# chhylp123/hifiasm

Measured on AMD Instinct MI355X. Metric: read-pair overlaps/sec (sum ol->length / (ha_pt_gen + all-reads h_ec_lchain pass)), higher is better.
Workload: dtype u64 hashing / int32 + f64 chain scores

## Files before the change

hifiasm_amd/csrc/hao_batch.hpp:

```cpp
#pragma once
#include <sys/mman.h>
#include "hao_tables.hpp"
#include "hao_query.cuh"
#include "hao_query3.cuh"
#include "hao_query5.cuh"
#include "hao_grid.cuh"
#include "hao_chain.cuh"

struct hao_ctx::Batch {
	uint64_t n_generic = 0, n_generic_hits = 0, seed_path = 0, seed_left[3] = {0, 0, 0}; DevBuf<unsigned long long> stats, dbgbuf;
	uint64_t lo = 0, n = 0, mz0 = 0, n_mz = 0, n_anchor = 0, n_groups = 0, n_chains = 0, n_cl = 0, n_fc_raw = 0, n_ol = 0, n_fc = 0, n_fcw = 0;
	bool valid = false, host_valid = false;
	DevBuf<uint64_t> s_start, s_pk, a_off, seg, g_cnt, g_off, g_start, ch_base, cl_base, fc_base, fcs, fc_raw, ol_fc_off, cc_off, cc, fc_final, fcf_off;
	DevBuf<uint64_t> nch64;
	DevBuf<uint64_t> g_tmp, cls_cc, cls_co; DevBuf<hao_gent> glist; DevBuf<uint8_t> g_cls; DevBuf<uint32_t> slow, ovf_list; hipStream_t side[HAO_NCLS]; hipEvent_t ev_qc[HAO_NCLS], ev_dp[HAO_NCLS]; bool side_ready = false; hipEvent_t ev_pk0 = nullptr, ev_pk1 = nullptr; DevBuf<unsigned char> pk_tmp;
	DevBuf<uint32_t> q_pos, q_cnt, s_n, g_read, wgt, nch, nout, perm, n_final, fclen;
	DevBuf<hao_hit_t> hits, ohits, cl;
	DevBuf<int32_t> f, ii, p, key_sc, tm; DevBuf<int64_t> t; DevBuf<uint64_t> key_xs; DevBuf<uint32_t> key_al, key_tmp;
	DevBuf<hao_chain_rec> rec; DevBuf<hao_ovlp_t> ol; DevBuf<hao_cdesc> cd; bool cl_valid = false;
	DevBuf<uint16_t> hq, ohq; DevBuf<uint8_t> hcode;
	DevBuf<uint32_t> pk_cnt, pk_ecnt, pk_erank; uint64_t n_codes = 0;
	struct OutSet {
		DevBuf<hao_ovlp_t> ol_out; DevBuf<hao_ovlp_wire_t> ol_wire; DevBuf<uint64_t> fin_off, fc_out, fc_out_off, ch_off, cl_off, qm_off, fcw_off; DevBuf<uint32_t> fcw;
		DevBuf<hao_chain_hdr_t> hdr; DevBuf<uint64_t> bits; DevBuf<uint32_t> rank, rank4; DevBuf<uint8_t> codes; DevBuf<hao_exc_t> exc; DevBuf<hao_qmz_t> qmz; DevBuf<uint16_t> qmz_pos, qmz_cnt; bool qmz16 = false;
		DevBuf<uint8_t> exact;
		DevBuf<uint64_t> ed_off; DevBuf<uint8_t> ed_err; DevBuf<uint16_t> ed_pe;
		DevBuf<hao_ed_ovlp_sum> ed_sum;
		DevBuf<uint64_t> wl_woff, wl_cigoff; DevBuf<hao_rs_win> wl_wins; DevBuf<uint16_t> wl_cig;
		DevBuf<hao_rs_ovlp> rs_ovlp; DevBuf<uint64_t> rs_off; DevBuf<hao_rs_win> rs_wins;
		DevBuf<uint64_t> tr_off; DevBuf<uint16_t> tr_ps, tr_ncig, tr_cig;
	} out[2];
	int cur = 0;
	OutSet &O() { return out[cur]; }
	unsigned char *arena[2] = { nullptr, nullptr }; size_t arena_cap[2] = { 0, 0 }; bool arena_reg[2] = { false, false };
	void arena_free(int x) { if (!arena[x]) return; if (arena_reg[x]) { (void)hipHostUnregister(arena[x]); (void)munmap(arena[x], arena_cap[x]); } else (void)hipHostFree(arena[x]); arena[x] = nullptr; arena_cap[x] = 0; arena_reg[x] = false; } hipStream_t copy_stream = nullptr; hipEvent_t ev_ready[2], ev_done[2], ev_cstart[2]; bool arena_bad[2] = { false, false }; int arena_retry[2] = { 0, 0 }, arena_node = -1;       bool dl_ready = false, dl_pending[2] = { false, false };
	uint32_t wgt_hi = 0xffffffffu, wgt_lo = 0xffffffffu, wgt_max = 0xffffffffu;
	double t_evsync = 0, t_enq = 0, t_alloc = 0, t_s1 = 0, t_s2 = 0, t_s3 = 0, t_run = 0, t_pre = 0; uint64_t t_n = 0, t_nrun = 0;
	uint64_t ed_unres = 0;
	DevBuf<uint64_t> ed_nwin, ed_wbase, ed_wcnt, ed_woff; DevBuf<hao_ed_pair> ed_pairs; uint64_t ed_n = 0;
	hao_ed_delivery_t ed_dl[2] = {};
	uint64_t wl_cnt[5] = { 0, 0, 0, 0, 0 }; hao_wlist_delivery_t wl_dl[2] = {}; bool wl_on[2] = { false, false };
	uint64_t rs_nw = 0, rs_nres = 0, rs_wc = 0; hao_rescue_delivery_t rs_dl[2] = {}; bool rs_on[2] = { false, false };
	uint64_t tr_n = 0, tr_ncig = 0; hao_trace_delivery_t tr_dl[2] = {}; bool tr_on[2] = { false, false };
	hao_delivery_t dl[2]; uint64_t dl_seq = 0, n_exc = 0; uint32_t dl_parts = 0; bool exact_valid = false; std::vector<uint8_t> h_exact;
	std::vector<uint64_t> h_seg, h_fin_off, h_cl_off, h_fc_out_off; std::vector<hao_hit_t> h_hits, h_cl; std::vector<hao_ovlp_t> h_ol; std::vector<uint64_t> h_fc;
	std::vector<uint64_t> fetch_fc_off, h_cco;
	~Batch() {
		if (ev_pk0) { (void)hipEventDestroy(ev_pk0); (void)hipEventDestroy(ev_pk1); }
		if (side_ready) { for (int x = 0; x < HAO_NCLS; ++x) { (void)hipStreamDestroy(side[x]); (void)hipEventDestroy(ev_qc[x]); (void)hipEventDestroy(ev_dp[x]); } }
		if (dl_ready) { (void)hipStreamSynchronize(copy_stream); (void)hipStreamDestroy(copy_stream); for (int x = 0; x < 2; ++x) { (void)hipEventDestroy(ev_ready[x]); (void)hipEventDestroy(ev_done[x]); (void)hipEventDestroy(ev_cstart[x]); arena_free(x); } }
	}
};

__global__ void hao_cc_count_kernel(const uint32_t *len, uint64_t rid0, uint64_t n, uint64_t ocv_w, uint64_t *out)
{
	const uint64_t r = (uint64_t)blockIdx.x * blockDim.x + threadIdx.x;
	if (r > n) return;
// ... 492 lines not shown
		HIP_TRY(hipMemcpy(c->h_ix_mz_off.data(), c->d_ix_mz_off.p, (c->n_reads + 1) * 8, hipMemcpyDeviceToHost));
	}
	const uint64_t glo = c->rid_base + lo;
	B.mz0 = c->h_ix_mz_off[lo]; B.n_mz = c->h_ix_mz_off[hi] - B.mz0;
	const uint64_t nm = B.n_mz;
	if (B.wgt_hi != ps.high_occ || B.wgt_lo != ps.low_occ || !B.wgt.p) {
		std::vector<uint32_t> wt; hao_seed_weight_table(ps.high_occ, ps.low_occ, wt);
		HIP_TRY(B.wgt.reserve(4096)); HIP_TRY(hipMemcpy(B.wgt.p, wt.data(), 4096 * 4, hipMemcpyHostToDevice));
		B.wgt_hi = ps.high_occ; B.wgt_lo = ps.low_occ; B.wgt_max = *std::max_element(wt.begin(), wt.end());
	}
	HIP_TRY(B.q_pos.reserve(nm + 1)); HIP_TRY(B.q_cnt.reserve(nm + 1));
	HIP_TRY(B.s_start.reserve(nm + 1)); HIP_TRY(B.s_pk.reserve(nm + 1)); HIP_TRY(B.s_n.reserve(nm + 1)); HIP_TRY(B.a_off.reserve(nm + 2)); HIP_TRY(B.seg.reserve(n + 2));
	HIP_TRY(c->d_err.reserve(2)); HIP_TRY(hipMemsetAsync(c->d_err.p, 0, 4, c->stream));
	if (!c->lk_valid) { hao_set_err(c, "index without per-minimizer lookup results"); return HAO_EINVAL; }
	hipLaunchKernelGGL(seed_unpack_kernel, dim3((unsigned)((nm + 256) / 256)), dim3(256), 0, c->stream, c->d_ix_lk.p, c->d_ix_mz_info.p, B.mz0, nm, B.wgt.p, B.s_start.p, B.s_n.p, B.q_pos.p, B.q_cnt.p, B.s_pk.p);
	HAO_CHECK_LAUNCH();
	if (int rc = hao_scan_u32(c, B.s_n.p, B.a_off.p, nm + 1)) return rc;
	hipLaunchKernelGGL(seed_segments_kernel, dim3((unsigned)((n + 256) / 256)), dim3(256), 0, c->stream, c->d_ix_mz_off.p, lo, n, B.mz0, B.a_off.p, B.seg.p);
	HAO_CHECK_LAUNCH();
	hipLaunchKernelGGL(hao_peek_kernel, dim3(1), dim3(64), 0, c->stream, (const unsigned long long*)(B.a_off.p + nm), 1, c->peek_d);
	HAO_CHECK_LAUNCH();
	const double ts0_ = hao_now();
	HIP_TRY(hipStreamSynchronize(c->stream));
	B.t_s1 += hao_now() - ts0_; B.t_pre += ts0_ - t_run0;
	B.n_anchor = c->peek_h[0];
	c->timer.mark("q_lookup");
	const uint64_t A = B.n_anchor;
	if (A >= (1ULL << 32)) { hao_set_err(c, "batch produces >= 2^32 anchors: use a smaller read range"); return HAO_EUNSUPP; }
	HIP_TRY(B.hits.reserve(A + 1));
	uint64_t max_q = 1;
	for (uint64_t r = lo; r < hi; ++r) max_q = std::max<uint64_t>(max_q, c->h_ix_mz_off[r + 1] - c->h_ix_mz_off[r]);
	const uint64_t sum_q = c->h_ix_mz_off[hi] - c->h_ix_mz_off[lo];
	int tb = 1; while ((1ULL << tb) < c->n_total) ++tb;
	HIP_TRY(B.g_cnt.reserve(n + 2)); HIP_TRY(B.g_off.reserve(n + 2)); HIP_TRY(B.g_tmp.reserve(A + 1));
	HIP_TRY(B.stats.reserve(3 * HAO_NCLS + 7)); HIP_TRY(hipMemsetAsync(B.stats.p, 0, (3 * HAO_NCLS + 7) * 8, c->stream));
	unsigned long long *d_slow_cnt = B.stats.p, *d_cls_cnt = B.stats.p + HAO_NCLS + 4;
	{
		hao_seed_args sa_; B.seed_path = 0;
		sa_.mz_off = c->d_ix_mz_off.p; sa_.mz_info = c->d_ix_mz_info.p; sa_.rid_lo = lo; sa_.mz0 = B.mz0; sa_.s_start = B.s_start.p; sa_.s_n = B.s_n.p; sa_.a_off = B.a_off.p; sa_.seg = B.seg.p;
		sa_.sinfo = c->d_ix_sinfo.p; sa_.len = c->d_len_all.p; sa_.q_pos = B.q_pos.p; sa_.q_cnt = B.q_cnt.p; sa_.hits = B.hits.p; sa_.g_tmp = B.g_tmp.p; sa_.g_cnt = B.g_cnt.p; sa_.n_sel = n; sa_.tb = tb;
		sa_.qcap = (uint32_t)std::min<uint64_t>((max_q + 63) & ~63ULL, HAO_QTAB_CAP);
		sa_.dbg = nullptr; sa_.hq = nullptr;
		if (parts & HAO_DELIVER_CL) {
			HIP_TRY(B.hcode.reserve(A + 64));
			if (c->sw.seq_chain || c->sw.dp_seqtail || c->sw.dp_nospec) { const uint64_t n16 = (A + 31) / 16; hipLaunchKernelGGL(hao_fill16_kernel, dim3((unsigned)std::min<uint64_t>((n16 + 255) / 256, 1u << 14)), dim3(256), 0, c->stream, (hao_fill_v4*)B.hcode.p, n16, 0x08080808u); HAO_CHECK_LAUNCH(); }
			HIP_TRY(B.hq.reserve(A + 64)); sa_.hq = B.hq.p;
		}
		if (c->sw.seedphase) { HIP_TRY(B.dbgbuf.reserve(64)); HIP_TRY(hipMemsetAsync(B.dbgbuf.p, 0, 512, c->stream)); sa_.dbg = B.dbgbuf.p; }
		HIP_TRY(B.ovf_list.reserve(3 * (n + 1)));
		unsigned long long *d_ovf = B.stats.p + 3 * HAO_NCLS + 3, *d_ovf2 = B.stats.p + 3 * HAO_NCLS + 4, *d_ovf0 = B.stats.p + 3 * HAO_NCLS + 5;
		uint32_t *ovf1 = B.ovf_list.p, *ovf2 = B.ovf_list.p + (n + 1), *ovf0 = B.ovf_list.p + 2 * (n + 1);
		const size_t lds_tile = std::max<size_t>((size_t)512 * (sizeof(hao_stage_t) + 4), 12 * 512);
		const size_t lds_q = 12 * (size_t)sa_.qcap + 16;
		size_t lds1 = (size_t)22 * 512 + lds_tile + lds_q, lds2 = (size_t)22 * 1024 + std::max<size_t>(lds_tile, 12 * 1024) + lds_q,
			   lds3 = (size_t)22 * 2048 + std::max<size_t>(lds_tile, 12 * 2048) + lds_q;
		auto launch = [&](auto k1, auto k2, auto k3) -> int {
			{
				HIP_TRY(hipFuncSetAttribute((const void*)k1, hipFuncAttributeMaxDynamicSharedMemorySize, (int)lds1));
				HIP_TRY(hipFuncSetAttribute((const void*)k2, hipFuncAttributeMaxDynamicSharedMemorySize, (int)lds2));
				HIP_TRY(hipFuncSetAttribute((const void*)k3, hipFuncAttributeMaxDynamicSharedMemorySize, (int)lds3));
			}
			hipLaunchKernelGGL(k1, dim3((unsigned)n), dim3(256), lds1, c->stream, sa_, (const uint32_t*)nullptr, (const unsigned long long*)nullptr, ovf1, d_ovf);
			HAO_CHECK_LAUNCH();
			hipLaunchKernelGGL(k2, dim3((unsigned)n), dim3(256), lds2, c->stream, sa_, (const uint32_t*)ovf1, (const unsigned long long*)d_ovf, ovf2, d_ovf2);
			HAO_CHECK_LAUNCH();
			hipLaunchKernelGGL(k3, dim3((unsigned)n), dim3(256), lds3, c->stream, sa_, (const uint32_t*)ovf2, (const unsigned long long*)d_ovf2, (uint32_t*)nullptr, (unsigned long long*)nullptr);
			HAO_CHECK_LAUNCH();
// ... 103 lines not shown
			const hao_gent *lst0 = B.glist.p + L.base[0]; uint32_t *slow0 = B.slow.p + L.base[0];
			const unsigned nb_lane = (unsigned)std::min<uint64_t>((cls_cnt[0] + 63) / 64, 256 * 64);
			if (ca.dbg_seq == 1) hipLaunchKernelGGL(chain_tiny_kernel, dim3(nb_lane), dim3(64), 0, c->stream, ca, lst0, (uint64_t)cls_cnt[0], (const uint32_t*)nullptr, (const unsigned long long*)nullptr);
			else {
				hipLaunchKernelGGL(chain_pack8_kernel, dim3((unsigned)((cls_cnt[0] + 31) / 32)), dim3(256), 0, c->stream, ca, lst0, (uint64_t)cls_cnt[0], slow0);
				HAO_CHECK_LAUNCH();
				hipLaunchKernelGGL(chain_tiny_kernel, dim3(nb_lane), dim3(64), 0, c->stream, ca, lst0, (uint64_t)cls_cnt[0], (const uint32_t*)slow0, (const unsigned long long*)d_slow_cnt);
			}
			HAO_CHECK_LAUNCH();
		}
		if (ca.dbg_qc) { unsigned long long d_[5]; HIP_TRY(hipMemcpy(d_, B.dbgbuf.p, 40, hipMemcpyDeviceToHost)); if (d_[3]) fprintf(stderr, "[qc] fast groups %llu (avg %.0f hits)  avg us: entry + tile 0 %.2f  scan loop %.2f  cigar + record %.2f\n", d_[3], (double)d_[4] / d_[3], d_[0] / 100.0 / d_[3], d_[1] / 100.0 / d_[3], d_[2] / 100.0 / d_[3]); }
		c->timer.mark("q_chain");
		if (!serial) for (int x = 1; x < HAO_NCLS; ++x) if (cls_cnt[x]) HIP_TRY(hipStreamWaitEvent(c->stream, B.ev_dp[x], 0));
	}
	HIP_TRY(hipMemsetAsync(B.nch.p + G, 0, 4, c->stream)); HIP_TRY(hipMemsetAsync(B.nout.p + G, 0, 4, c->stream));
	c->timer.mark("q_chain_dp");
	HIP_TRY(B.ch_base.reserve(G + 2)); HIP_TRY(B.cl_base.reserve(G + 2)); HIP_TRY(B.fc_base.reserve(G * HAO_MCOPY_MAX + 2)); HIP_TRY(B.nch64.reserve(G * HAO_MCOPY_MAX + 2));
	if (int rc = hao_scan_u32(c, B.nch.p, B.ch_base.p, G + 1)) return rc;
	if (int rc = hao_scan_u32(c, B.nout.p, B.cl_base.p, G + 1)) return rc;
	hipLaunchKernelGGL(hao_fclen_kernel, dim3((unsigned)((G * HAO_MCOPY_MAX + 256) / 256)), dim3(256), 0, c->stream, B.rec.p, B.nch.p, G, B.nch64.p);
	HAO_CHECK_LAUNCH();
	if (int rc = hao_excl_scan_u64(c, B.nch64.p, B.fc_base.p, G * HAO_MCOPY_MAX + 1)) return rc;
	const uint64_t NCmax = G * HAO_MCOPY_MAX, FCmax = A + 6 * G;
	HIP_TRY(B.ol.reserve(NCmax + 1)); HIP_TRY(B.ol_fc_off.reserve(NCmax + 1)); HIP_TRY(B.cd.reserve(NCmax + 1)); HIP_TRY(B.fc_raw.reserve(FCmax + 1)); HIP_TRY(B.perm.reserve(NCmax + 1));
	if (G) {
		hao_asm_args aa;
		aa.g_start = B.g_start.p; aa.g_read = B.g_read.p; aa.g_cls = B.g_cls.p; aa.g_off = B.g_off.p; aa.n_groups = G; aa.rid_lo = glo; aa.ohits = B.ohits.p; aa.hits = B.hits.p; aa.fcs = B.fcs.p; aa.rec = B.rec.p; aa.nch = B.nch.p;
		aa.ch_base = B.ch_base.p; aa.cl_base = B.cl_base.p; aa.fc_base = B.fc_base.p; aa.ol = B.ol.p; aa.ol_fc_off = B.ol_fc_off.p; aa.cd = B.cd.p; aa.fc = B.fc_raw.p;
		hipLaunchKernelGGL(chain_assemble_kernel, dim3((unsigned)((G + 255) / 256)), dim3(256), 0, c->stream, aa); HAO_CHECK_LAUNCH();
	}
	unsigned long long *d_exc_cnt = B.stats.p + 3 * HAO_NCLS + 2;
	hao_pack_args pa; memset(&pa, 0, sizeof(pa));
	const uint64_t NW = (A + 63) / 64;
	unsigned long long *d_n_codes = B.stats.p + 3 * HAO_NCLS + 1;
	auto pack = [&](hipStream_t ps) -> int {
		if (!G) return HAO_OK;
		hao_ctx::Batch::OutSet &O = B.O();
		hipLaunchKernelGGL(hao_pack_hdr_kernel, dim3((unsigned)((NCmax + 255) / 256)), dim3(256), 0, ps, pa, B.ch_base.p + G); HAO_CHECK_LAUNCH();
		hipLaunchKernelGGL(hao_pack_bits_kernel, dim3((unsigned)((NW * 8 + 256 * HAO_PACK_U - 1) / (256 * HAO_PACK_U))), dim3(256), 0, ps, pa, A, NW, O.bits.p, B.pk_cnt.p, B.pk_ecnt.p); HAO_CHECK_LAUNCH();
		size_t tb = 0;
		HIP_TRY(rocprim::exclusive_scan(nullptr, tb, B.pk_cnt.p, O.rank.p, 0u, NW + 1, rocprim::plus<uint32_t>(), ps)); HIP_TRY(B.pk_tmp.reserve(tb + 256));
		HIP_TRY(rocprim::exclusive_scan(B.pk_tmp.p, tb, B.pk_cnt.p, O.rank.p, 0u, NW + 1, rocprim::plus<uint32_t>(), ps));
		HIP_TRY(rocprim::exclusive_scan(B.pk_tmp.p, tb, B.pk_ecnt.p, B.pk_erank.p, 0u, NW + 1, rocprim::plus<uint32_t>(), ps));
		hipLaunchKernelGGL(hao_pack_codes_kernel, dim3((unsigned)((NW * 8 + 255) / 256)), dim3(256), 0, ps, pa, B.hcode.p, A, O.bits.p, O.rank.p, NW, O.codes.p, d_n_codes, B.pk_erank.p); HAO_CHECK_LAUNCH();
		{ const uint64_t n4 = NW / 4 + 1; hipLaunchKernelGGL(hao_rank4_kernel, dim3((unsigned)((n4 + 255) / 256)), dim3(256), 0, ps, O.rank.p, n4, O.rank4.p); HAO_CHECK_LAUNCH(); }
		return HAO_OK;
	};
	bool pack_on_side = false;
	if (parts & HAO_DELIVER_CL) {
		hao_ctx::Batch::OutSet &O = B.O();
		HIP_TRY(O.hdr.reserve(NCmax + 1)); HIP_TRY(O.exc.reserve(c->sw.exc_cap >= 0 ? (uint64_t)c->sw.exc_cap + 1 : std::max<uint64_t>(1 << 14, A / 256)));
		HIP_TRY(O.bits.reserve(NW + 2)); HIP_TRY(O.rank.reserve(NW + 6)); HIP_TRY(O.rank4.reserve(NW / 4 + 2)); HIP_TRY(B.pk_cnt.reserve(NW + 2)); HIP_TRY(O.codes.reserve(A + 16));
		HIP_TRY(B.pk_ecnt.reserve(NW + 2)); HIP_TRY(B.pk_erank.reserve(NW + 2));
		HIP_TRY(O.ch_off.reserve(n + 2)); HIP_TRY(O.cl_off.reserve(n + 2)); HIP_TRY(O.qm_off.reserve(n + 2));
		O.qmz16 = c->max_len_all < 65536 && B.wgt_max < 256 && !c->sw.qmz_raw;
		if (O.qmz16) { HIP_TRY(O.qmz_pos.reserve(nm + 1)); HIP_TRY(O.qmz_cnt.reserve(nm + 1)); } else HIP_TRY(O.qmz.reserve(nm + 1));
		pa.cd = B.cd.p; pa.hits = B.hits.p; pa.ohits = B.ohits.p; pa.mz_off = c->d_ix_mz_off.p; pa.seg = B.seg.p; pa.n_sel = n; pa.rid_lo = lo; pa.mz0 = B.mz0; pa.q_pos = B.q_pos.p;
		pa.hq = B.hq.p; pa.ohq = B.ohq.p;
		pa.hdr = O.hdr.p; pa.bytes = B.hcode.p; pa.exc = O.exc.p; pa.exc_cnt = d_exc_cnt; pa.exc_every = (uint32_t)c->sw.exc_every;
		pa.exc_cap = c->sw.exc_cap >= 0 ? std::min<uint64_t>(O.exc.cap, (uint64_t)c->sw.exc_cap) : O.exc.cap;
		hipStream_t ps = c->stream;
		if (B.side_ready && !c->sw.dp_serial) {
			if (!B.ev_pk0) { HIP_TRY(hipEventCreateWithFlags(&B.ev_pk0, hipEventDisableTiming)); HIP_TRY(hipEventCreateWithFlags(&B.ev_pk1, hipEventDisableTiming)); }
			ps = B.side[0]; pack_on_side = true;
			HIP_TRY(hipEventRecord(B.ev_pk0, c->stream)); HIP_TRY(hipStreamWaitEvent(ps, B.ev_pk0, 0));
		}
		HIP_TRY(hipMemsetAsync(B.pk_cnt.p + NW, 0, 4, ps));
		HIP_TRY(hipMemsetAsync(B.pk_ecnt.p + NW, 0, 4, ps));
		if (int rc = pack(ps)) return rc;
		hipLaunchKernelGGL(hao_read_ranges_kernel, dim3((unsigned)((n + 256) / 256)), dim3(256), 0, ps, B.g_off.p, B.ch_base.p, B.cl_base.p, c->d_ix_mz_off.p, lo, B.mz0, n, O.ch_off.p, O.cl_off.p, O.qm_off.p);
		HAO_CHECK_LAUNCH();
		if (nm && O.qmz16) { hipLaunchKernelGGL(hao_qtab16_kernel, dim3((unsigned)((nm + 255) / 256)), dim3(256), 0, ps, B.q_pos.p, B.q_cnt.p, nm, O.qmz_pos.p, O.qmz_cnt.p, c->d_err.p); HAO_CHECK_LAUNCH(); }
		else if (nm) { hipLaunchKernelGGL(hao_qtab_kernel, dim3((unsigned)((nm + 255) / 256)), dim3(256), 0, ps, B.q_pos.p, B.q_cnt.p, nm, O.qmz.p); HAO_CHECK_LAUNCH(); }
		if (pack_on_side) HIP_TRY(hipEventRecord(B.ev_pk1, ps));
	}
	c->timer.mark("q_assemble");
	{
		uint64_t o = 0;
		for (uint64_t r = 0; r < n; ++r) o += c->h_len_all[glo + r] / par.ocv_w + 2;
		HIP_TRY(B.cc_off.reserve(n + 2)); HIP_TRY(B.cc.reserve(o + 1)); HIP_TRY(B.n_final.reserve(n + 2)); HIP_TRY(B.fc_final.reserve(n + 2));
		HIP_TRY(B.O().fin_off.reserve(n + 2)); HIP_TRY(B.fcf_off.reserve(n + 2)); HIP_TRY(B.nch64.reserve(n + 2));
		hipLaunchKernelGGL(hao_cc_count_kernel, dim3((unsigned)((n + 256) / 256)), dim3(256), 0, c->stream, c->d_len_all.p, glo, n, (uint64_t)par.ocv_w, B.nch64.p);
		HAO_CHECK_LAUNCH();
		if (int rc = hao_excl_scan_u64(c, B.nch64.p, B.cc_off.p, n + 1)) return rc;
	}
	const uint64_t NC = NCmax;
	HIP_TRY(B.key_xs.reserve(NC + 1)); HIP_TRY(B.key_sc.reserve(NC + 1)); HIP_TRY(B.key_al.reserve(NC + 1));
	hao_sel_args sa;
	HIP_TRY(B.key_tmp.reserve(5 * NC + 8));
	sa.key_xs = B.key_xs.p; sa.key_sc = B.key_sc.p; sa.key_al = B.key_al.p; sa.key_tmp = B.key_tmp.p;
	sa.ol = B.ol.p; sa.g_off = B.g_off.p; sa.ch_base = B.ch_base.p; sa.cl_base = B.cl_base.p; sa.cd = B.cd.p; sa.hits = B.hits.p; sa.ohits = B.ohits.p; sa.n_sel = n; sa.rid_lo = glo; sa.len = c->d_len_all.p; sa.cc_off = B.cc_off.p; sa.cc = B.cc.p;
	sa.perm = B.perm.p; sa.n_final = B.n_final.p; sa.fc_final = B.fc_final.p; sa.max_n_chain = par.max_n_chain; sa.ocv_w = par.ocv_w; sa.chain_cutoff = par.chain_cutoff;
	sa.dbg = nullptr; sa.dbg_seq_prune = c->sw.seq_prune ? 1 : 0;
	if (c->sw.selphase) { HIP_TRY(B.dbgbuf.reserve(8)); HIP_TRY(hipMemsetAsync(B.dbgbuf.p, 0, 64, c->stream)); sa.dbg = B.dbgbuf.p; }
	hipLaunchKernelGGL((chain_select_kernel<1, 128>), dim3((unsigned)(n + 1)), dim3(64), 0, c->stream, sa, (int64_t)0, (int64_t)129);
	HAO_CHECK_LAUNCH();
	{
		hipLaunchKernelGGL((chain_select4_kernel<512>), dim3((unsigned)n), dim3(256), 0, c->stream, sa, (int64_t)129, (int64_t)513);
		HAO_CHECK_LAUNCH();
		hipLaunchKernelGGL((chain_select4_kernel<1024>), dim3((unsigned)n), dim3(256), 0, c->stream, sa, (int64_t)513, (int64_t)1025);
		HAO_CHECK_LAUNCH();
// ... 9 lines not shown
	if (sa.dbg) { unsigned long long d_[5]; HIP_TRY(hipMemcpy(d_, B.dbgbuf.p, 40, hipMemcpyDeviceToHost)); if (d_[4]) fprintf(stderr, "[select] reads %llu  avg us: score sort %.1f  prune %.1f  position sort %.1f  weak filter %.1f\n", d_[4], d_[0] / 100.0 / d_[4], d_[1] / 100.0 / d_[4], d_[2] / 100.0 / d_[4], d_[3] / 100.0 / d_[4]); }
	c->timer.mark("q_select");
	HIP_TRY(B.O().ol_out.reserve(NCmax + 1)); HIP_TRY(B.O().fc_out.reserve(FCmax + 1)); HIP_TRY(B.O().fc_out_off.reserve(NCmax + 2));
	unsigned long long *d_n_fcw = B.stats.p + 3 * HAO_NCLS;
	const bool fcw_ = (parts & HAO_DELIVER_OL) != 0;
	if (fcw_) { HIP_TRY(B.O().fcw_off.reserve(NCmax + 2)); HIP_TRY(B.O().fcw.reserve(3 * (FCmax + 1))); HIP_TRY(B.O().ol_wire.reserve(NCmax + 1)); }
	hipLaunchKernelGGL(chain_final_kernel, dim3((unsigned)((n + 3) / 4)), dim3(256), 0, c->stream, B.ol.p, B.ol_fc_off.p, B.fc_raw.p, B.perm.p, B.g_off.p, B.ch_base.p,
					   B.O().fin_off.p, B.fcf_off.p, n, B.O().ol_out.p, B.O().fc_out.p, B.O().fc_out_off.p, fcw_ ? B.O().fcw.p : (uint32_t*)nullptr, fcw_ ? B.O().fcw_off.p : (uint64_t*)nullptr, d_n_fcw, (uint32_t)c->sw.fc_raw_every);
	HAO_CHECK_LAUNCH();
	if (fcw_) { hipLaunchKernelGGL(hao_ol_wire_kernel, dim3((unsigned)std::min<uint64_t>((NCmax + 255) / 256, 4096)), dim3(256), 0, c->stream, B.O().ol_out.p, B.O().fin_off.p + n, B.O().ol_wire.p); HAO_CHECK_LAUNCH(); }
	if (pack_on_side) HIP_TRY(hipStreamWaitEvent(c->stream, B.ev_pk1, 0));
	c->timer.mark("q_final");
	unsigned long long slow_st[HAO_NCLS + 4], n_exc = 0;
	{
		auto peek = [&](const void *src, int nw, int at) { hipLaunchKernelGGL(hao_peek_kernel, dim3(1), dim3(64), 0, c->stream, (const unsigned long long*)src, nw, c->peek_d + at); };
		peek(B.ch_base.p + G, 1, 0); peek(B.cl_base.p + G, 1, 1); peek(B.fc_base.p + G * HAO_MCOPY_MAX, 1, 2); peek(B.O().fin_off.p + n, 1, 3); peek(B.fcf_off.p + n, 1, 4);
		peek(d_slow_cnt, HAO_NCLS + 4, 8); peek(d_exc_cnt, 1, 5); peek(d_n_codes, 1, 6); peek(d_n_fcw, 1, 7); peek(B.stats.p + 3 * HAO_NCLS + 3, 3, 24); peek(c->d_err.p, 1, 27);
		HAO_CHECK_LAUNCH();
		const double ts2_ = hao_now();
		HIP_TRY(hipStreamSynchronize(c->stream));
		B.t_s3 += hao_now() - ts2_; B.t_run += hao_now() - t_run0; ++B.t_nrun;
		if (c->sw.dltime && (B.t_nrun & 15) == 0) fprintf(stderr, "[batch] %llu runs (parts %u): total %.1f ms  before sync1 %.1f  sync1 %.1f  sync2 %.1f  sync3 %.1f\n", (unsigned long long)B.t_nrun, parts, B.t_run * 1e3, B.t_pre * 1e3, B.t_s1 * 1e3, B.t_s2 * 1e3, B.t_s3 * 1e3);
		B.n_chains = c->peek_h[0]; B.n_cl = c->peek_h[1]; B.n_fc_raw = c->peek_h[2]; B.n_ol = c->peek_h[3]; B.n_fc = c->peek_h[4];
		for (int x = 0; x < HAO_NCLS + 4; ++x) slow_st[x] = c->peek_h[8 + x];
		B.seed_left[0] = c->peek_h[26]; B.seed_left[1] = c->peek_h[24]; B.seed_left[2] = c->peek_h[25];
		if (parts & HAO_DELIVER_CL) { n_exc = c->peek_h[5]; B.n_codes = G ? c->peek_h[6] : 0; }
		if ((parts & HAO_DELIVER_CL) && (uint32_t)c->peek_h[27]) { hao_set_err(c, "a minimizer position or seed weight that does not fit the packed minimizer table"); return HAO_EUNSUPP; }
		if ((parts & HAO_DELIVER_OL) && (c->peek_h[7] >> 63)) { hao_set_err(c, "an overlap without fake-cigar entries: the packed cigar layout holds at least one per overlap"); return HAO_EUNSUPP; }
		B.n_fcw = (parts & HAO_DELIVER_OL) ? (B.n_fc - B.n_ol) + c->peek_h[7] : 0;
	}
	if ((parts & HAO_DELIVER_CL) && n_exc > pa.exc_cap) {
		HIP_TRY(B.O().exc.reserve(n_exc + 1024)); pa.exc = B.O().exc.p; pa.exc_cap = B.O().exc.cap;
		HIP_TRY(hipMemsetAsync(d_exc_cnt, 0, 8, c->stream));
		HIP_TRY(hipMemsetAsync(B.pk_cnt.p + NW, 0, 4, c->stream)); HIP_TRY(hipMemsetAsync(B.pk_ecnt.p + NW, 0, 4, c->stream));
		if (int rc = pack(c->stream)) return rc;
		hipLaunchKernelGGL(hao_peek_kernel, dim3(1), dim3(64), 0, c->stream, (const unsigned long long*)d_exc_cnt, 1, c->peek_d + 5); HAO_CHECK_LAUNCH();
		hipLaunchKernelGGL(hao_peek_kernel, dim3(1), dim3(64), 0, c->stream, (const unsigned long long*)d_n_codes, 1, c->peek_d + 6); HAO_CHECK_LAUNCH();
		HIP_TRY(hipStreamSynchronize(c->stream));
		B.n_codes = c->peek_h[6];
		n_exc = c->peek_h[5];
	}
	B.n_exc = n_exc;
	B.n_generic = 0; for (int x = 0; x < HAO_NCLS; ++x) B.n_generic += slow_st[x];
	B.n_generic_hits = slow_st[HAO_NCLS];
	if (c->sw.dp_stats) { fprintf(stderr, "[dp] slow groups by class:"); for (int x = 0; x < HAO_NCLS; ++x) fprintf(stderr, " %llu/%llu", slow_st[x], cls_cnt[x]);
		fprintf(stderr, "  hits %llu  dp range %llu  spec-committed %llu  spec-failures %llu\n", slow_st[HAO_NCLS], slow_st[HAO_NCLS + 3], slow_st[HAO_NCLS + 1], slow_st[HAO_NCLS + 2]); }
	B.valid = true;
	if (parts & HAO_DELIVER_EXACT) { if (int rc = hao_exact_run(c)) return rc; }
	if (parts & HAO_DELIVER_ED) { if (int rc = hao_ed_deliver_run(c)) return rc; }
	if (parts & HAO_DELIVER_TRACE) { if (int rc = hao_trace_deliver_run(c)) return rc; }
	if (parts & HAO_DELIVER_RESCUE) { if (int rc = hao_rescue_deliver_run(c)) return rc; }
	if (parts & HAO_DELIVER_WLIST) { if (int rc = hao_wlist_deliver_run(c)) return rc; }
	if (parts) { const double t0_ = hao_now(); const int rc_ = hao_deliver_enqueue(c); B.t_enq += hao_now() - t0_; ++B.t_n; if (c->sw.dltime && (B.t_n & 15) == 0) fprintf(stderr, "[deliver] %llu batches: slot wait %.1f ms, enqueue %.1f ms (arena alloc %.1f ms)\n", (unsigned long long)B.t_n, B.t_evsync * 1e3, B.t_enq * 1e3, B.t_alloc * 1e3); return rc_; }
	return HAO_OK;
}

static int hao_batch_materialize_cl(hao_ctx *c)
{
	hao_ctx::Batch &B = *c->batch;
	if (B.cl_valid) return HAO_OK;
	HIP_TRY(B.cl.reserve(B.n_cl + 1));
	if (B.n_chains) {
		hipLaunchKernelGGL(chain_materialize_kernel, dim3((unsigned)((B.n_chains + 3) / 4)), dim3(256), 0, c->stream, B.cd.p, B.n_chains, B.hits.p, B.ohits.p, B.cl.p);
		HAO_CHECK_LAUNCH();
		HIP_TRY(hipStreamSynchronize(c->stream));
	}
	B.cl_valid = true;
// ... 31 lines not shown
```

hifiasm_amd/csrc/hao_deliver.cuh:

```cuda
#pragma once
#include "hao_common.cuh"
#include "hao_chain.cuh"

__host__ __device__ __forceinline__ uint64_t hao_dg_mix(uint64_t z)
{ z ^= z >> 30; z *= 0xbf58476d1ce4e5b9ULL; z ^= z >> 27; z *= 0x94d049bb133111ebULL; z ^= z >> 31; return z; }
__host__ __device__ __forceinline__ uint64_t hao_dg_term(uint64_t stream, uint64_t i, uint64_t w)
{ return hao_dg_mix(w + 0x9E3779B97F4A7C15ULL * (i + 1) + stream * 0xD6E8FEB86659FD93ULL); }

struct hao_digest_args {
	const uint64_t *fin_off, *fcf_off, *g_off, *cl_base, *seg;
	const uint64_t *ol, *fc, *cl, *hits;
	uint64_t n_sel; uint64_t *dig, *dig_kh;
};

__device__ __forceinline__ uint64_t hao_dg_range(uint64_t stream, const uint64_t *w, uint64_t n_words, uint32_t tid)
{
	uint64_t s = 0;
	for (uint64_t i = tid; i < n_words; i += 256) s += hao_dg_term(stream, i, w[i]);
	return s;
}

__global__ __launch_bounds__(256) void hao_digest_kernel(hao_digest_args A)
{
	const uint64_t r = blockIdx.x; const uint32_t tid = threadIdx.x;
// ... 7 lines not shown
	if ((tid & 63) == 0) { part[0][tid >> 6] = d; part[1][tid >> 6] = k; }
	__syncthreads();
	if (tid == 0) {
		A.dig[r] = part[0][0] + part[0][1] + part[0][2] + part[0][3];
		if (A.dig_kh) A.dig_kh[r] = part[1][0] + part[1][1] + part[1][2] + part[1][3];
	}
}

#define HAO_PACK_QCAP 1024
struct hao_pack_args {
	const hao_cdesc *cd; const hao_hit_t *hits, *ohits;
	const uint64_t *mz_off, *seg; uint64_t rid_lo, mz0, n_sel; const uint32_t *q_pos;
	hao_chain_hdr_t *hdr; uint8_t *bytes; hao_exc_t *exc; unsigned long long *exc_cnt; uint64_t exc_cap; uint32_t exc_every;
	const uint16_t *hq;
	const uint16_t *ohq;
};

__device__ __forceinline__ uint32_t hao_pack_find_q(const uint32_t *qp, uint32_t nq, uint32_t self_offset)
{ uint32_t lo = 0, hi = nq; while (lo < hi) { const uint32_t m = (lo + hi) >> 1; if (qp[m] < self_offset) lo = m + 1; else hi = m; } return lo; }

__global__ __launch_bounds__(256) void hao_pack_hdr_kernel(hao_pack_args A, const uint64_t *n_chains_dev)
{
	const uint64_t ci = (uint64_t)blockIdx.x * 256 + threadIdx.x;
	if (ci >= *n_chains_dev) return;
	const hao_cdesc d = A.cd[ci];
	const hao_hit_t h0 = hao_cd_src(d, A.hits, A.ohits)[0];
	const uint64_t pos = d.src & ~HAO_CD_OHITS;
	uint32_t q0 = A.hq ? ((d.src & HAO_CD_OHITS) ? (A.ohq ? A.ohq[pos] : 65535u) : A.hq[pos]) : 65535u;
	if (q0 == 65535u) { const uint64_t m0 = A.mz_off[A.rid_lo + d.r]; q0 = hao_pack_find_q(A.q_pos + (m0 - A.mz0), (uint32_t)(A.mz_off[A.rid_lo + d.r + 1] - m0), h0.self_offset); }
	hao_chain_hdr_t H; H.n_hits = d.n; H.w0 = d.w0; H.q0 = q0; H.offset = h0.offset; H.pos = pos;
	A.hdr[ci] = H;
}

#define HAO_PACK_U 4
static_assert(HAO_CODE_EXC_OHITS == 0xfd, "hao_pack_bits_kernel tests the byte 0xfd");
__device__ __forceinline__ uint32_t hao_byte_flags(uint64_t hi_bits) { return (uint32_t)(((hi_bits >> 7) * 0x0102040810204080ULL) >> 56); }
__global__ __launch_bounds__(256) void hao_pack_bits_kernel(hao_pack_args A, uint64_t n, uint64_t n_words, uint64_t *bits, uint32_t *cnt, uint32_t *ecnt)
{
	const uint64_t T = (uint64_t)gridDim.x * 256, t0 = (uint64_t)blockIdx.x * 256 + threadIdx.x;
	const uint64_t L7 = 0x7f7f7f7f7f7f7f7fULL, H8 = 0x8080808080808080ULL;
	uint64_t v[HAO_PACK_U];
#pragma unroll
	for (int u = 0; u < HAO_PACK_U; ++u) { const uint64_t t = t0 + (uint64_t)u * T; v[u] = 8 * t < n ? *(const uint64_t*)(A.bytes + 8 * t) : 0x0808080808080808ULL; }
#pragma unroll
	for (int u = 0; u < HAO_PACK_U; ++u) {
		const uint64_t t = t0 + (uint64_t)u * T, w = t >> 3;
		const uint64_t x = v[u] ^ 0x0808080808080808ULL, xf = ~v[u], xd = v[u] ^ 0xfdfdfdfdfdfdfdfdULL;
		uint32_t m8 = hao_byte_flags((x | ((x & L7) + L7)) & H8);
		uint32_t e8 = hao_byte_flags((~(((xf & L7) + L7) | xf | L7) | ~(((xd & L7) + L7) | xd | L7)) & H8);
		const uint64_t left = 8 * t < n ? n - 8 * t : 0;
		if (left < 8) { const uint32_t keep = (1u << (uint32_t)left) - 1u; m8 &= keep; e8 &= keep; }
		if (w < n_words) ((uint8_t*)bits)[t] = (uint8_t)m8;
		uint32_t pc = (uint32_t)__popc(m8) | (uint32_t)__popc(e8) << 16;
		pc += (uint32_t)hao_dpp<0x101, 0xf>(0, (int)pc); pc += (uint32_t)hao_dpp<0x102, 0xf>(0, (int)pc); pc += (uint32_t)hao_dpp<0x104, 0xf>(0, (int)pc);
		if ((t & 7) == 0 && w < n_words) { cnt[w] = pc & 0xffffu; ecnt[w] = pc >> 16; }
	}
}

__global__ __launch_bounds__(256) void hao_pack_codes_kernel(hao_pack_args A, const uint8_t *bytes, uint64_t n, const uint64_t *bits, const uint32_t *rank, uint64_t n_words, uint8_t *codes,
		unsigned long long *n_codes, const uint32_t *erank)
{
	const uint64_t t = (uint64_t)blockIdx.x * 256 + threadIdx.x, w = t >> 3;
	if (t == 0) { *n_codes = rank[n_words]; *A.exc_cnt = erank[n_words]; }
	const bool in = 8 * t < n;
	const uint64_t word = in ? bits[w] : 0; const int sh = (int)(t & 7) * 8;
	uint32_t m8 = (uint32_t)(word >> sh) & 0xffu, e8 = 0;
	uint64_t v = 0;
	if (m8) v = *(const uint64_t*)(bytes + 8 * t);
	if (m8) {
		uint64_t at = rank[w] + (uint64_t)__popcll(word & ((1ULL << sh) - 1));
		for (uint32_t m = m8; m; m &= m - 1) { const uint8_t b = (uint8_t)(v >> (8 * (__ffs((int)m) - 1))); codes[at++] = b >= HAO_CODE_EXC_OHITS ? (uint8_t)0xff : b; }
	}
	for (uint32_t m = m8; m; m &= m - 1) { const int k = __ffs((int)m) - 1; const uint8_t b = (uint8_t)(v >> (8 * k)); if (b == 0xff || b == HAO_CODE_EXC_OHITS) e8 |= 1u << k; }
	uint64_t eword = (uint64_t)e8 << sh;
	eword |= __shfl_xor(eword, 1); eword |= __shfl_xor(eword, 2); eword |= __shfl_xor(eword, 4);
	if (!e8) return;
	unsigned long long kx = (unsigned long long)erank[w] + (unsigned long long)__popcll(eword & ((1ULL << sh) - 1));
	for (uint32_t m = e8; m; m &= m - 1, ++kx) {
		if (kx >= A.exc_cap) continue;
		const uint64_t p = 8 * t + (uint32_t)(__ffs((int)m) - 1);
		const bool oh = (uint8_t)(v >> (8 * (__ffs((int)m) - 1))) == HAO_CODE_EXC_OHITS;
		hao_exc_t e; e.index = p; e.pad = 0; e.hit = oh ? A.ohits[p] : A.hits[p]; e.q = oh ? A.ohq[p] : (A.hq ? A.hq[p] : 65535u);
		if (e.q == 65535u) {
			uint64_t lo = 0, hi = A.n_sel; while (hi - lo > 1) { const uint64_t md = (lo + hi) >> 1; if (A.seg[md] <= p) lo = md; else hi = md; }
			const uint64_t m0 = A.mz_off[A.rid_lo + lo];
			e.q = hao_pack_find_q(A.q_pos + (m0 - A.mz0), (uint32_t)(A.mz_off[A.rid_lo + lo + 1] - m0), e.hit.self_offset);
		}
		A.exc[kx] = e;
	}
}

__global__ void hao_rank4_kernel(const uint32_t *rank, uint64_t n4, uint32_t *out)
{
	const uint64_t i = (uint64_t)blockIdx.x * blockDim.x + threadIdx.x;
	if (i < n4) out[i] = rank[4 * i];
}


typedef uint32_t hao_fill_v4 __attribute__((ext_vector_type(4)));
__global__ __launch_bounds__(256) void hao_fill16_kernel(hao_fill_v4 *p, uint64_t n16, uint32_t word)
{
	const hao_fill_v4 v = { word, word, word, word };
	for (uint64_t i = (uint64_t)blockIdx.x * 256 + threadIdx.x; i < n16; i += (uint64_t)gridDim.x * 256) p[i] = v;
}

__global__ __launch_bounds__(256) void hao_ol_wire_kernel(const hao_ovlp_t *ol, const uint64_t *n_dev, hao_ovlp_wire_t *out)
{
	const uint64_t n = *n_dev;
	for (uint64_t i = (uint64_t)blockIdx.x * 256 + threadIdx.x; i < n; i += (uint64_t)gridDim.x * 256) {
		const hao_ovlp_t o = ol[i]; hao_ovlp_wire_t w;
		w.y = o.y_id | o.y_pos_strand << 31; w.x_pos_s = o.x_pos_s; w.x_pos_e = o.x_pos_e; w.y_pos_s = o.y_pos_s; w.y_pos_e = o.y_pos_e;
		w.shared_seed = o.shared_seed; w.non_homopolymer_errors = o.non_homopolymer_errors; w.fc_len = o.fc_len;
		out[i] = w;
	}
}

__global__ void hao_qtab_kernel(const uint32_t *q_pos, const uint32_t *q_cnt, uint64_t n_mz, hao_qmz_t *out)
{
	const uint64_t i = (uint64_t)blockIdx.x * blockDim.x + threadIdx.x;
	if (i < n_mz) { hao_qmz_t v; v.self_offset = q_pos[i]; v.cnt = q_cnt[i]; out[i] = v; }
}

__global__ void hao_qtab16_kernel(const uint32_t *q_pos, const uint32_t *q_cnt, uint64_t n_mz, uint16_t *pos, uint16_t *cnt, int *err)
{
	const uint64_t i = (uint64_t)blockIdx.x * blockDim.x + threadIdx.x;
	if (i < n_mz) { const uint32_t p = q_pos[i], k = q_cnt[i]; pos[i] = (uint16_t)p; cnt[i] = (uint16_t)k; if (p > 0xffffu || k > 0xffffu) *err = 1; }
}

// ... 71 lines not shown
```

Measured before the change: 179.8 million.

## Replace per-word pack pipeline with block sweep, staged compaction, and placement kernels

The pack stage used to build a bitmap plus per-word code and exception counts, run two NW-length scans, then scatter codes and build rank4 in separate kernels. It now compacts each 8K-position block's flagged bytes in shared memory during the sweep and stages them in g_tmp. A single scan over per-block totals (packed into u64) follows, and one place kernel copies the staged run, writes rank4 and emits exceptions. This cuts scan length, kernel launches, memsets and the full rank array, in exchange for a staging buffer and block-local scans with more complex indexing.

```diff
diff --git a/hifiasm_amd/csrc/hao_batch.hpp b/hifiasm_amd/csrc/hao_batch.hpp
--- a/hifiasm_amd/csrc/hao_batch.hpp
+++ b/hifiasm_amd/csrc/hao_batch.hpp
@@ -19,10 +19,10 @@
 	DevBuf<int32_t> f, ii, p, key_sc, tm; DevBuf<int64_t> t; DevBuf<uint64_t> key_xs; DevBuf<uint32_t> key_al, key_tmp;
 	DevBuf<hao_chain_rec> rec; DevBuf<hao_ovlp_t> ol; DevBuf<hao_cdesc> cd; bool cl_valid = false;
 	DevBuf<uint16_t> hq, ohq; DevBuf<uint8_t> hcode;
-	DevBuf<uint32_t> pk_cnt, pk_ecnt, pk_erank; uint64_t n_codes = 0;
+	DevBuf<uint64_t> pk_tot, pk_base; uint64_t n_codes = 0;
 	struct OutSet {
 		DevBuf<hao_ovlp_t> ol_out; DevBuf<hao_ovlp_wire_t> ol_wire; DevBuf<uint64_t> fin_off, fc_out, fc_out_off, ch_off, cl_off, qm_off, fcw_off; DevBuf<uint32_t> fcw;
-		DevBuf<hao_chain_hdr_t> hdr; DevBuf<uint64_t> bits; DevBuf<uint32_t> rank, rank4; DevBuf<uint8_t> codes; DevBuf<hao_exc_t> exc; DevBuf<hao_qmz_t> qmz; DevBuf<uint16_t> qmz_pos, qmz_cnt; bool qmz16 = false;
+		DevBuf<hao_chain_hdr_t> hdr; DevBuf<uint64_t> bits; DevBuf<uint32_t> rank4; DevBuf<uint8_t> codes; DevBuf<hao_exc_t> exc; DevBuf<hao_qmz_t> qmz; DevBuf<uint16_t> qmz_pos, qmz_cnt; bool qmz16 = false;
 		DevBuf<uint8_t> exact;
 		DevBuf<uint64_t> ed_off; DevBuf<uint8_t> ed_err; DevBuf<uint16_t> ed_pe;
 		DevBuf<hao_ed_ovlp_sum> ed_sum;
@@ -581,7 +581,7 @@
 	for (uint64_t r = lo; r < hi; ++r) max_q = std::max<uint64_t>(max_q, c->h_ix_mz_off[r + 1] - c->h_ix_mz_off[r]);
 	const uint64_t sum_q = c->h_ix_mz_off[hi] - c->h_ix_mz_off[lo];
 	int tb = 1; while ((1ULL << tb) < c->n_total) ++tb;
-	HIP_TRY(B.g_cnt.reserve(n + 2)); HIP_TRY(B.g_off.reserve(n + 2)); HIP_TRY(B.g_tmp.reserve(A + 1));
+	HIP_TRY(B.g_cnt.reserve(n + 2)); HIP_TRY(B.g_off.reserve(n + 2)); HIP_TRY(B.g_tmp.reserve(std::max<uint64_t>(A + 1, A / 8 + HAO_SWEEP_POS / 8 + 2)));
 	HIP_TRY(B.stats.reserve(3 * HAO_NCLS + 7)); HIP_TRY(hipMemsetAsync(B.stats.p, 0, (3 * HAO_NCLS + 7) * 8, c->stream));
 	unsigned long long *d_slow_cnt = B.stats.p, *d_cls_cnt = B.stats.p + HAO_NCLS + 4;
 	{
@@ -751,26 +751,26 @@
 	unsigned long long *d_exc_cnt = B.stats.p + 3 * HAO_NCLS + 2;
 	hao_pack_args pa; memset(&pa, 0, sizeof(pa));
 	const uint64_t NW = (A + 63) / 64;
+	const uint64_t NB = (A + HAO_SWEEP_POS - 1) / HAO_SWEEP_POS;
 	unsigned long long *d_n_codes = B.stats.p + 3 * HAO_NCLS + 1;
 	auto pack = [&](hipStream_t ps) -> int {
 		if (!G) return HAO_OK;
 		hao_ctx::Batch::OutSet &O = B.O();
 		hipLaunchKernelGGL(hao_pack_hdr_kernel, dim3((unsigned)((NCmax + 255) / 256)), dim3(256), 0, ps, pa, B.ch_base.p + G); HAO_CHECK_LAUNCH();
-		hipLaunchKernelGGL(hao_pack_bits_kernel, dim3((unsigned)((NW * 8 + 256 * HAO_PACK_U - 1) / (256 * HAO_PACK_U))), dim3(256), 0, ps, pa, A, NW, O.bits.p, B.pk_cnt.p, B.pk_ecnt.p); HAO_CHECK_LAUNCH();
+		uint8_t *stage = (uint8_t*)B.g_tmp.p;
+		hipLaunchKernelGGL(hao_pack_sweep_kernel, dim3((unsigned)NB), dim3(256), 0, ps, (const uint8_t*)B.hcode.p, A, NW, O.bits.p, stage, B.pk_tot.p); HAO_CHECK_LAUNCH();
 		size_t tb = 0;
-		HIP_TRY(rocprim::exclusive_scan(nullptr, tb, B.pk_cnt.p, O.rank.p, 0u, NW + 1, rocprim::plus<uint32_t>(), ps)); HIP_TRY(B.pk_tmp.reserve(tb + 256));
-		HIP_TRY(rocprim::exclusive_scan(B.pk_tmp.p, tb, B.pk_cnt.p, O.rank.p, 0u, NW + 1, rocprim::plus<uint32_t>(), ps));
-		HIP_TRY(rocprim::exclusive_scan(B.pk_tmp.p, tb, B.pk_ecnt.p, B.pk_erank.p, 0u, NW + 1, rocprim::plus<uint32_t>(), ps));
-		hipLaunchKernelGGL(hao_pack_codes_kernel, dim3((unsigned)((NW * 8 + 255) / 256)), dim3(256), 0, ps, pa, B.hcode.p, A, O.bits.p, O.rank.p, NW, O.codes.p, d_n_codes, B.pk_erank.p); HAO_CHECK_LAUNCH();
-		{ const uint64_t n4 = NW / 4 + 1; hipLaunchKernelGGL(hao_rank4_kernel, dim3((unsigned)((n4 + 255) / 256)), dim3(256), 0, ps, O.rank.p, n4, O.rank4.p); HAO_CHECK_LAUNCH(); }
+		HIP_TRY(rocprim::exclusive_scan(nullptr, tb, B.pk_tot.p, B.pk_base.p, (uint64_t)0, NB, rocprim::plus<uint64_t>(), ps)); HIP_TRY(B.pk_tmp.reserve(tb + 256));
+		HIP_TRY(rocprim::exclusive_scan(B.pk_tmp.p, tb, B.pk_tot.p, B.pk_base.p, (uint64_t)0, NB, rocprim::plus<uint64_t>(), ps));
+		hipLaunchKernelGGL(hao_pack_place_kernel, dim3((unsigned)NB), dim3(256), 0, ps, pa, NW, (const uint64_t*)O.bits.p, (const uint8_t*)stage, (const uint64_t*)B.pk_tot.p, (const uint64_t*)B.pk_base.p, O.codes.p, O.rank4.p, d_n_codes); HAO_CHECK_LAUNCH();
 		return HAO_OK;
 	};
 	bool pack_on_side = false;
 	if (parts & HAO_DELIVER_CL) {
 		hao_ctx::Batch::OutSet &O = B.O();
 		HIP_TRY(O.hdr.reserve(NCmax + 1)); HIP_TRY(O.exc.reserve(c->sw.exc_cap >= 0 ? (uint64_t)c->sw.exc_cap + 1 : std::max<uint64_t>(1 << 14, A / 256)));
-		HIP_TRY(O.bits.reserve(NW + 2)); HIP_TRY(O.rank.reserve(NW + 6)); HIP_TRY(O.rank4.reserve(NW / 4 + 2)); HIP_TRY(B.pk_cnt.reserve(NW + 2)); HIP_TRY(O.codes.reserve(A + 16));
-		HIP_TRY(B.pk_ecnt.reserve(NW + 2)); HIP_TRY(B.pk_erank.reserve(NW + 2));
+		HIP_TRY(O.bits.reserve(NW + 2)); HIP_TRY(O.rank4.reserve(NW / 4 + 2)); HIP_TRY(O.codes.reserve(A + 16));
+		HIP_TRY(B.pk_tot.reserve(NB + 2)); HIP_TRY(B.pk_base.reserve(NB + 2));
 		HIP_TRY(O.ch_off.reserve(n + 2)); HIP_TRY(O.cl_off.reserve(n + 2)); HIP_TRY(O.qm_off.reserve(n + 2));
 		O.qmz16 = c->max_len_all < 65536 && B.wgt_max < 256 && !c->sw.qmz_raw;
 		if (O.qmz16) { HIP_TRY(O.qmz_pos.reserve(nm + 1)); HIP_TRY(O.qmz_cnt.reserve(nm + 1)); } else HIP_TRY(O.qmz.reserve(nm + 1));
@@ -784,8 +784,6 @@
 			ps = B.side[0]; pack_on_side = true;
 			HIP_TRY(hipEventRecord(B.ev_pk0, c->stream)); HIP_TRY(hipStreamWaitEvent(ps, B.ev_pk0, 0));
 		}
-		HIP_TRY(hipMemsetAsync(B.pk_cnt.p + NW, 0, 4, ps));
-		HIP_TRY(hipMemsetAsync(B.pk_ecnt.p + NW, 0, 4, ps));
 		if (int rc = pack(ps)) return rc;
 		hipLaunchKernelGGL(hao_read_ranges_kernel, dim3((unsigned)((n + 256) / 256)), dim3(256), 0, ps, B.g_off.p, B.ch_base.p, B.cl_base.p, c->d_ix_mz_off.p, lo, B.mz0, n, O.ch_off.p, O.cl_off.p, O.qm_off.p);
 		HAO_CHECK_LAUNCH();
@@ -861,7 +859,6 @@
 	if ((parts & HAO_DELIVER_CL) && n_exc > pa.exc_cap) {
 		HIP_TRY(B.O().exc.reserve(n_exc + 1024)); pa.exc = B.O().exc.p; pa.exc_cap = B.O().exc.cap;
 		HIP_TRY(hipMemsetAsync(d_exc_cnt, 0, 8, c->stream));
-		HIP_TRY(hipMemsetAsync(B.pk_cnt.p + NW, 0, 4, c->stream)); HIP_TRY(hipMemsetAsync(B.pk_ecnt.p + NW, 0, 4, c->stream));
 		if (int rc = pack(c->stream)) return rc;
 		hipLaunchKernelGGL(hao_peek_kernel, dim3(1), dim3(64), 0, c->stream, (const unsigned long long*)d_exc_cnt, 1, c->peek_d + 5); HAO_CHECK_LAUNCH();
 		hipLaunchKernelGGL(hao_peek_kernel, dim3(1), dim3(64), 0, c->stream, (const unsigned long long*)d_n_codes, 1, c->peek_d + 6); HAO_CHECK_LAUNCH();
diff --git a/hifiasm_amd/csrc/hao_deliver.cuh b/hifiasm_amd/csrc/hao_deliver.cuh
--- a/hifiasm_amd/csrc/hao_deliver.cuh
+++ b/hifiasm_amd/csrc/hao_deliver.cuh
@@ -63,54 +63,90 @@
 	A.hdr[ci] = H;
 }
 
-#define HAO_PACK_U 4
-static_assert(HAO_CODE_EXC_OHITS == 0xfd, "hao_pack_bits_kernel tests the byte 0xfd");
+#define HAO_SWEEP_U 4
+#define HAO_SWEEP_CHUNKS (256 * HAO_SWEEP_U)
+#define HAO_SWEEP_POS (8 * HAO_SWEEP_CHUNKS)
+static_assert(HAO_SWEEP_POS % 256 == 0 && HAO_SWEEP_POS < 65536, "a block is whole directory entries, and its two counts travel in the halves of one register");
+static_assert(HAO_CODE_EXC_OHITS == 0xfd, "hao_pack_sweep_kernel tests the byte 0xfd");
 __device__ __forceinline__ uint32_t hao_byte_flags(uint64_t hi_bits) { return (uint32_t)(((hi_bits >> 7) * 0x0102040810204080ULL) >> 56); }
-__global__ __launch_bounds__(256) void hao_pack_bits_kernel(hao_pack_args A, uint64_t n, uint64_t n_words, uint64_t *bits, uint32_t *cnt, uint32_t *ecnt)
-{
-	const uint64_t T = (uint64_t)gridDim.x * 256, t0 = (uint64_t)blockIdx.x * 256 + threadIdx.x;
+__global__ __launch_bounds__(256) void hao_pack_sweep_kernel(const uint8_t *bytes, uint64_t n, uint64_t n_words, uint64_t *bits, uint8_t *stage, uint64_t *tot)
+{
+	__shared__ uint32_t part[HAO_SWEEP_U * 4];
+	__shared__ uint64_t run[HAO_SWEEP_POS / 8];
+	const uint32_t tid = threadIdx.x, wv = tid >> 6; const uint64_t c0 = (uint64_t)blockIdx.x * HAO_SWEEP_CHUNKS + tid;
 	const uint64_t L7 = 0x7f7f7f7f7f7f7f7fULL, H8 = 0x8080808080808080ULL;
-	uint64_t v[HAO_PACK_U];
-#pragma unroll
-	for (int u = 0; u < HAO_PACK_U; ++u) { const uint64_t t = t0 + (uint64_t)u * T; v[u] = 8 * t < n ? *(const uint64_t*)(A.bytes + 8 * t) : 0x0808080808080808ULL; }
-#pragma unroll
-	for (int u = 0; u < HAO_PACK_U; ++u) {
-		const uint64_t t = t0 + (uint64_t)u * T, w = t >> 3;
+	uint64_t v[HAO_SWEEP_U]; uint32_t m8[HAO_SWEEP_U], ex[HAO_SWEEP_U];
+#pragma unroll
+	for (int u = 0; u < HAO_SWEEP_U; ++u) { const uint64_t t = c0 + (uint64_t)u * 256; v[u] = 8 * t < n ? *(const uint64_t*)(bytes + 8 * t) : 0x0808080808080808ULL; }
+#pragma unroll
+	for (int u = 0; u < HAO_SWEEP_U; ++u) {
+		const uint64_t t = c0 + (uint64_t)u * 256;
 		const uint64_t x = v[u] ^ 0x0808080808080808ULL, xf = ~v[u], xd = v[u] ^ 0xfdfdfdfdfdfdfdfdULL;
-		uint32_t m8 = hao_byte_flags((x | ((x & L7) + L7)) & H8);
+		uint32_t m = hao_byte_flags((x | ((x & L7) + L7)) & H8);
 		uint32_t e8 = hao_byte_flags((~(((xf & L7) + L7) | xf | L7) | ~(((xd & L7) + L7) | xd | L7)) & H8);
 		const uint64_t left = 8 * t < n ? n - 8 * t : 0;
-		if (left < 8) { const uint32_t keep = (1u << (uint32_t)left) - 1u; m8 &= keep; e8 &= keep; }
-		if (w < n_words) ((uint8_t*)bits)[t] = (uint8_t)m8;
-		uint32_t pc = (uint32_t)__popc(m8) | (uint32_t)__popc(e8) << 16;
-		pc += (uint32_t)hao_dpp<0x101, 0xf>(0, (int)pc); pc += (uint32_t)hao_dpp<0x102, 0xf>(0, (int)pc); pc += (uint32_t)hao_dpp<0x104, 0xf>(0, (int)pc);
-		if ((t & 7) == 0 && w < n_words) { cnt[w] = pc & 0xffffu; ecnt[w] = pc >> 16; }
-	}
-}
-
-__global__ __launch_bounds__(256) void hao_pack_codes_kernel(hao_pack_args A, const uint8_t *bytes, uint64_t n, const uint64_t *bits, const uint32_t *rank, uint64_t n_words, uint8_t *codes,
-		unsigned long long *n_codes, const uint32_t *erank)
-{
-	const uint64_t t = (uint64_t)blockIdx.x * 256 + threadIdx.x, w = t >> 3;
-	if (t == 0) { *n_codes = rank[n_words]; *A.exc_cnt = erank[n_words]; }
-	const bool in = 8 * t < n;
-	const uint64_t word = in ? bits[w] : 0; const int sh = (int)(t & 7) * 8;
-	uint32_t m8 = (uint32_t)(word >> sh) & 0xffu, e8 = 0;
-	uint64_t v = 0;
-	if (m8) v = *(const uint64_t*)(bytes + 8 * t);
-	if (m8) {
-		uint64_t at = rank[w] + (uint64_t)__popcll(word & ((1ULL << sh) - 1));
-		for (uint32_t m = m8; m; m &= m - 1) { const uint8_t b = (uint8_t)(v >> (8 * (__ffs((int)m) - 1))); codes[at++] = b >= HAO_CODE_EXC_OHITS ? (uint8_t)0xff : b; }
-	}
-	for (uint32_t m = m8; m; m &= m - 1) { const int k = __ffs((int)m) - 1; const uint8_t b = (uint8_t)(v >> (8 * k)); if (b == 0xff || b == HAO_CODE_EXC_OHITS) e8 |= 1u << k; }
-	uint64_t eword = (uint64_t)e8 << sh;
-	eword |= __shfl_xor(eword, 1); eword |= __shfl_xor(eword, 2); eword |= __shfl_xor(eword, 4);
-	if (!e8) return;
-	unsigned long long kx = (unsigned long long)erank[w] + (unsigned long long)__popcll(eword & ((1ULL << sh) - 1));
-	for (uint32_t m = e8; m; m &= m - 1, ++kx) {
+		if (left < 8) { const uint32_t keep = (1u << (uint32_t)left) - 1u; m &= keep; e8 &= keep; }
+		if ((t >> 3) < n_words) ((uint8_t*)bits)[t] = (uint8_t)m;
+		const uint32_t pc = (uint32_t)__popc(m) | (uint32_t)__popc(e8) << 16;
+		const uint32_t inc = hao_wave_incl_scan_u32(pc);
+		if ((tid & 63) == 63) part[u * 4 + wv] = inc;
+		m8[u] = m; ex[u] = inc - pc;
+	}
+	__syncthreads();
+	uint32_t before = 0, total = 0;
+#pragma unroll
+	for (int u = 0; u < HAO_SWEEP_U; ++u) {
+		uint32_t at = before;
+#pragma unroll
+		for (int w = 0; w < 4; ++w) { const uint32_t p = part[u * 4 + w]; if ((uint32_t)w < wv) at += p; before += p; }
+		at = (at + ex[u]) & 0xffffu;
+		for (uint32_t m = m8[u]; m; m &= m - 1) ((uint8_t*)run)[at++] = (uint8_t)(v[u] >> (8 * (__ffs((int)m) - 1)));
+	}
+	total = before;
+	__syncthreads();
+	const uint32_t nflag = total & 0xffffu;
+	uint64_t *out = (uint64_t*)(stage + (uint64_t)blockIdx.x * HAO_SWEEP_POS);
+	for (uint32_t i = tid; i < (nflag + 7) / 8; i += 256) out[i] = run[i];
+	if (tid == 0) tot[blockIdx.x] = (uint64_t)nflag | (uint64_t)(total >> 16) << 32;
+}
+
+__device__ __forceinline__ uint32_t hao_block_excl_scan_u32(uint32_t x, uint32_t *part, uint32_t tid)
+{
+	const uint32_t inc = hao_wave_incl_scan_u32(x);
+	if ((tid & 63) == 63) part[tid >> 6] = inc;
+	__syncthreads();
+	uint32_t at = inc - x;
+	for (uint32_t w = 0; w < (tid >> 6); ++w) at += part[w];
+	return at;
+}
+__global__ __launch_bounds__(256) void hao_pack_place_kernel(hao_pack_args A, uint64_t n_words, const uint64_t *bits, const uint8_t *stage, const uint64_t *tot, const uint64_t *base,
+		uint8_t *codes, uint32_t *rank4, unsigned long long *n_codes)
+{
+	__shared__ uint32_t part[2][4];
+	const uint32_t tid = threadIdx.x; const uint64_t b = blockIdx.x;
+	const uint64_t bs = base[b], ts = tot[b];
+	const uint64_t cbase = (uint32_t)bs, ebase = bs >> 32; const uint32_t nflag = (uint32_t)ts, nexc = (uint32_t)(ts >> 32);
+	const uint64_t n4 = n_words / 4 + 1;
+	if (b + 1 == gridDim.x && tid == 0) {
+		*n_codes = cbase + nflag; *A.exc_cnt = ebase + nexc;
+		if (n_words % (HAO_SWEEP_POS / 64) == 0) rank4[n_words / 4] = (uint32_t)(cbase + nflag);
+	}
+	const uint8_t *run = stage + b * HAO_SWEEP_POS;
+	for (uint32_t j = tid; j < nflag; j += 256) { const uint8_t c = run[j]; codes[cbase + j] = c >= HAO_CODE_EXC_OHITS ? (uint8_t)0xff : c; }
+	const uint64_t w = b * (HAO_SWEEP_POS / 64) + (tid >> 1);
+	const uint32_t h = w < n_words ? (uint32_t)(bits[w] >> (32 * (tid & 1))) : 0u;
+	const uint32_t fpre = hao_block_excl_scan_u32((uint32_t)__popc(h), part[0], tid);
+	const uint64_t i4 = b * (HAO_SWEEP_POS / 256) + (tid >> 3);
+	if ((tid & 7) == 0 && i4 < n4) rank4[i4] = (uint32_t)(cbase + fpre);
+	if (!nexc) return;
+	uint32_t vm = 0, om = 0, j = fpre;
+	for (uint32_t m = h; m; m &= m - 1, ++j) { const uint8_t c = run[j]; if (c == 0xff || c == HAO_CODE_EXC_OHITS) vm |= m & (0u - m); if (c == HAO_CODE_EXC_OHITS) om |= m & (0u - m); }
+	unsigned long long kx = ebase + hao_block_excl_scan_u32((uint32_t)__popc(vm), part[1], tid);
+	for (uint32_t m = vm; m; m &= m - 1, ++kx) {
 		if (kx >= A.exc_cap) continue;
-		const uint64_t p = 8 * t + (uint32_t)(__ffs((int)m) - 1);
-		const bool oh = (uint8_t)(v >> (8 * (__ffs((int)m) - 1))) == HAO_CODE_EXC_OHITS;
+		const uint32_t k = (uint32_t)(__ffs((int)m) - 1);
+		const uint64_t p = b * HAO_SWEEP_POS + 32 * (uint64_t)tid + k;
+		const bool oh = (om >> k) & 1u;
 		hao_exc_t e; e.index = p; e.pad = 0; e.hit = oh ? A.ohits[p] : A.hits[p]; e.q = oh ? A.ohq[p] : (A.hq ? A.hq[p] : 65535u);
 		if (e.q == 65535u) {
 			uint64_t lo = 0, hi = A.n_sel; while (hi - lo > 1) { const uint64_t md = (lo + hi) >> 1; if (A.seg[md] <= p) lo = md; else hi = md; }
@@ -119,12 +155,6 @@
 		}
 		A.exc[kx] = e;
 	}
-}
-
-__global__ void hao_rank4_kernel(const uint32_t *rank, uint64_t n4, uint32_t *out)
-{
-	const uint64_t i = (uint64_t)blockIdx.x * blockDim.x + threadIdx.x;
-	if (i < n4) out[i] = rank[4 * i];
 }
 
 
```

Result: no change. 180.9 million (median of 4 runs) (+0.6%).
